# Yxxxb/LAVT-RS

Measured on AMD Instinct MI355X. Metric: train images/sec (480x480 Swin-B LAVT, fwd+bwd), higher is better.
Workload: dtype bf16; 1 GPU; swin_b_w12_480_b2; global_batch=2, image=480, n_l=20, parallelism=dp1, hip_graph=True, loss_kernel=fused upsample+CE

## Files before the change

lavt-rs_amd/csrc/gemm_tn_pipe.hip:

```cpp
#include "gemm_v2_helpers.h"
#include "internal.h"
#include "ln_bwd_body.h"

namespace {

typedef i32x8 __attribute__((aligned(4))) tnp_i32x8_u;
typedef __attribute__((address_space(4))) const tnp_i32x8_u* tnp_cptr8;
typedef __attribute__((address_space(4))) const int* tnp_cptr1;

template <int OFF> __device__ __forceinline__ void tnp_rd1(unsigned a, u64& d) {
    asm volatile("ds_read_b64_tr_b16 %0, %1 offset:%c2" : "=&v"(d) : "v"(a), "n"(OFF) : "memory");
}
__device__ __forceinline__ void tnp_tie1(u64& l, u64& h) { asm volatile("" : "+v"(l), "+v"(h)); }

constexpr int TNP_MAX = 6;
enum { TNP_ACCUMULATE = 1, TNP_COLSUM_ATOMIC = 2, TNP_NO_B = 4, TNP_VEC4 = 8, TNP_PART_VEC4 = 16, TNP_WT = 32 };
struct TnpMember {
    const bf16* A; const bf16* B; float* C; float* colsum;
    const int32_t* a_map; const int32_t* b_map; const float* a_rs;
    int64_t ldc;
    int lda, ldb, I, J, K, tiles_j, tile_end, rs_div, rs_n, flags;
    float alpha;
    float* part;
    int pieces, kt_per, tiles;
// ... 254 lines not shown
#undef TNP_MFMA_ONE

    const float alpha = m.alpha;
    const bool to_part = m.pieces > 1;
    float* const Cp = to_part ? m.part + (int64_t)piece * m.I * m.J : m.C;
    const int64_t ldc = to_part ? m.J : m.ldc;
    const bool accum = !to_part && (m.flags & TNP_ACCUMULATE), vec4 = to_part ? (m.flags & TNP_PART_VEC4) != 0 : (m.flags & TNP_VEC4) != 0;
    const bool wt = !to_part && (m.flags & TNP_WT) != 0;
    if (has_b) {
#pragma unroll
        for (int fi = 0; fi < 4; ++fi) {
            const int ii = i0 + wi * 64 + fi * 16 + l15;
#pragma unroll
            for (int fj = 0; fj < 2; ++fj) {
                const int jj = j0 + wj * 32 + fj * 16 + 4 * g4;
                if (ii < m.I && jj < m.J) {
                    float* dst = Cp + (int64_t)ii * ldc + jj;
                    float4 v = make_float4(alpha * acc[fi][fj][0], alpha * acc[fi][fj][1], alpha * acc[fi][fj][2], alpha * acc[fi][fj][3]);
                    if (vec4) {
                        if (accum) { const float4 o = *reinterpret_cast<const float4*>(dst); v.x += o.x; v.y += o.y; v.z += o.z; v.w += o.w; }
                        if (wt) st16_out(dst, make_uint4(__float_as_uint(v.x), __float_as_uint(v.y), __float_as_uint(v.z), __float_as_uint(v.w)));
                        else *reinterpret_cast<float4*>(dst) = v;
                    } else {
                        if (accum) { v.x += dst[0]; v.y += dst[1]; v.z += dst[2]; v.w += dst[3]; }
                        dst[0] = v.x; dst[1] = v.y; dst[2] = v.z; dst[3] = v.w;
                    }
                }
            }
        }
    }
    if (cs_wave && g4 == 0) {
        const bool cat = !to_part && ((m.flags & TNP_COLSUM_ATOMIC) || accum);
        float* const csb = to_part ? m.part + (int64_t)m.pieces * m.I * m.J + (int64_t)piece * m.I : m.colsum;
#pragma unroll
        for (int fi = 0; fi < 4; ++fi) {
            const int ii = i0 + wi * 64 + fi * 16 + l15;
            if (ii < m.I) {
                float* cs = csb + ii;
                if (cat) atomicAdd(cs, alpha * cacc[fi][0]); else *cs = alpha * cacc[fi][0];
            }
        }
    }
}

template <int STAGES, int LPR>
__global__ __launch_bounds__(512) void gemm_tn_pipe_kernel(const TnpGroup g, const TnpRider ln) {
    extern __shared__ __attribute__((aligned(16))) char smem[];
    const int bid = blockIdx.x;
    if (bid >= g.tiles) {
        if constexpr (LPR > 0) {
            int unit = 2 * (bid - g.tiles) + (int)(threadIdx.x >> 8);
            unit = unit < ln.blocks ? unit : ln.blocks - 1;
            layernorm_bwd_body<bf16, LPR, 1, 4, 0>(ln.dy, ln.x, nullptr, ln.gamma, ln.mean, ln.rstd, ln.dx, nullptr, nullptr, ln.partials, ln.dres, ln.rows, ln.C, nullptr,
                                                   nullptr, unit, ln.blocks, (int)(threadIdx.x & 255), reinterpret_cast<float*>(smem + (threadIdx.x >> 8) * 16384));
        }
        return;
    }
    const int t = bid;
    int k = 0;
    while (k + 1 < g.n && t >= g.m[k].tile_end) ++k;
    const TnpMember& m = g.m[k];
    const int local = t - (k ? g.m[k - 1].tile_end : 0);
    if ((m.a_map || m.b_map) && (m.K & 7)) tnp_tile<STAGES, 2>(m, local, smem);
    else if (m.a_map || m.b_map || m.a_rs) tnp_tile<STAGES, 1>(m, local, smem);
    else tnp_tile<STAGES, 0>(m, local, smem);
}

__global__ __launch_bounds__(256) void tnp_reduce_pieces(const TnpGroup g) {
    const TnpMember& m = g.m[blockIdx.y];
    const int ns = m.pieces;
    if (ns <= 1) return;
    const int64_t W = (int64_t)m.I * m.J, total = W + (m.colsum ? m.I : 0);
    const int64_t e0 = ((int64_t)blockIdx.x * 256 + threadIdx.x) * 4;
    if (e0 >= total) return;
    const bool no_b = (m.flags & TNP_NO_B) != 0;
    const bool v4 = !no_b && (m.flags & TNP_PART_VEC4) && (m.flags & TNP_VEC4) && (m.J % 4 == 0);
    if (v4 && e0 + 3 < W) {
        const float* q = m.part + e0;
        float4 a0 = make_float4(0.f, 0.f, 0.f, 0.f), a1 = a0, a2 = a0, a3 = a0;
        int s = 0;
        for (; s + 7 < ns; s += 8) {
            float4 v[8];
#pragma unroll
            for (int u = 0; u < 8; ++u) v[u] = *reinterpret_cast<const float4*>(q + (int64_t)(s + u) * W);
#pragma unroll
            for (int u = 0; u < 8; u += 4) {
                a0.x += v[u].x; a0.y += v[u].y; a0.z += v[u].z; a0.w += v[u].w; a1.x += v[u + 1].x; a1.y += v[u + 1].y; a1.z += v[u + 1].z; a1.w += v[u + 1].w;
                a2.x += v[u + 2].x; a2.y += v[u + 2].y; a2.z += v[u + 2].z; a2.w += v[u + 2].w; a3.x += v[u + 3].x; a3.y += v[u + 3].y; a3.z += v[u + 3].z; a3.w += v[u + 3].w;
            }
        }
        if (s < ns) {
            float4 v[7];
#pragma unroll
            for (int u = 0; u < 7; ++u) v[u] = *reinterpret_cast<const float4*>(q + (int64_t)min(s + u, ns - 1) * W);
#pragma unroll
            for (int u = 0; u < 7; ++u)
                if (s + u < ns) { a0.x += v[u].x; a0.y += v[u].y; a0.z += v[u].z; a0.w += v[u].w; }
        }
        const int64_t i = e0 / m.J;
        float4* c = reinterpret_cast<float4*>(m.C + i * m.ldc + (e0 - i * m.J));
        float4 o = *c;
        o.x += (a0.x + a1.x) + (a2.x + a3.x); o.y += (a0.y + a1.y) + (a2.y + a3.y); o.z += (a0.z + a1.z) + (a2.z + a3.z); o.w += (a0.w + a1.w) + (a2.w + a3.w);
        *c = o;
        return;
    }
    for (int k = 0; k < 4; ++k) {
        const int64_t e = e0 + k;
// ... 100 lines not shown
```

lavt-rs_amd/csrc/gemm_tn_v2.hip:

```cpp
#include "gemm_v2_helpers.h"
#include "internal.h"
#include "ln_bwd_body.h"

namespace {

__device__ __forceinline__ void dma4(const void* src, void* lds_dst) {
    __builtin_amdgcn_global_load_lds((gbl_void*)src, (lds_void*)lds_dst, 4, 0, 0);
}

struct TnOut {
    float* C;
    int64_t ldc;
    float* colsum;
    bool atomic, colsum_atomic;
};
template <int BI, int BJ, int WAVES, int STAGES, bool MAPS, int CS, bool CONVP = true>
__device__ __forceinline__ void tn_tile_range(const lavt_gemm_tn_t& p, const int tile_linear, const int bz, const int kt_begin, const int kt_end, const TnOut o, char* smem) {
    using T = bf16;
    constexpr int BK = 64, EPC = 8;
    constexpr int WAVES_I = 2, WAVES_J = WAVES / WAVES_I;
    constexpr int A_CH = BI / EPC, B_CH = BJ / EPC;
    constexpr int A_INSTR = BK * A_CH / (64 * WAVES), B_INSTR = BK * B_CH / (64 * WAVES);
    static_assert(A_INSTR * 64 * WAVES == BK * A_CH && B_INSTR * 64 * WAVES == BK * B_CH, "whole DMA instructions per operand tile");
    constexpr int A_BYTES = A_INSTR * WAVES * 1024, B_BYTES = B_INSTR * WAVES * 1024, STAGE_BYTES = A_BYTES + B_BYTES;
// ... 297 lines not shown
    const bool to_parts = p.partials != nullptr && nsplit > 1;
    float* const pbase = to_parts ? p.partials + (int64_t)bz * nsplit * ((int64_t)p.I * p.J + p.I) : nullptr;
    TnOut o;
    o.C = to_parts ? pbase + (int64_t)split_idx * p.I * p.J : p.C + (int64_t)bz * p.strideC;
    o.ldc = to_parts ? p.J : p.ldc;
    o.colsum = to_parts ? pbase + (int64_t)nsplit * p.I * p.J + (int64_t)split_idx * p.I : (p.colsum ? p.colsum + (int64_t)bz * p.strideColsum : nullptr);
    o.atomic = !to_parts && (nsplit > 1 || p.accumulate);
    o.colsum_atomic = p.colsum_atomic && !to_parts;
    tn_tile_range<BI, BJ, WAVES, STAGES, MAPS, CS, CONVP>(p, tile_linear, bz, kt_begin, kt_end, o, smem);
}

template <int BI, int BJ, int WAVES, int STAGES, bool MAPS, int CS, bool CONVP = true>
__global__ __launch_bounds__(WAVES * 64) void gemm_tn_v2_kernel(const lavt_gemm_tn_t p, int kt_per_split) {
    extern __shared__ __attribute__((aligned(16))) char smem[];
    tn_tile<BI, BJ, WAVES, STAGES, MAPS, CS, CONVP>(p, blockIdx.x, blockIdx.y, blockIdx.z, kt_per_split, gridDim.z, smem);
}

constexpr int TN_GROUP_MAX = 6;
struct TnGroup {
    lavt_gemm_tn_t p[TN_GROUP_MAX];
    int tile_end[TN_GROUP_MAX];
    int split[TN_GROUP_MAX];
    int n;
};
template <int BI, int BJ, int WAVES, int STAGES, bool MAPS, int CS>
__device__ __forceinline__ void grouped_tile(const TnGroup& g, const int bid, char* smem) {
    int k = 0;
    while (k + 1 < g.n && bid >= g.tile_end[k]) ++k;
    const int local = bid - (k ? g.tile_end[k - 1] : 0);
    const lavt_gemm_tn_t& p = g.p[k];
    const int ns = g.split[k], ktiles = (p.K + 63) / 64;
    if constexpr (MAPS) {
        if (!(p.a_rowmap || p.a_rowscale || p.b_rowmap)) {
            tn_tile<BI, BJ, WAVES, STAGES, false, CS, false>(p, local / ns, 0, local % ns, (ktiles + ns - 1) / ns, ns, smem);
            return;
        }
    }
    tn_tile<BI, BJ, WAVES, STAGES, MAPS, CS, false>(p, local / ns, 0, local % ns, (ktiles + ns - 1) / ns, ns, smem);
}
template <int BI, int BJ, int WAVES, int STAGES, bool MAPS, int CS>
__global__ __launch_bounds__(WAVES * 64, (BI == 128 && WAVES == 8) ? 4 : 1) void gemm_tn_v2_grouped_kernel(const TnGroup g) {
    extern __shared__ __attribute__((aligned(16))) char smem[];
    grouped_tile<BI, BJ, WAVES, STAGES, MAPS, CS>(g, blockIdx.x, smem);
}
struct LnRider {
    const bf16* dy; const bf16* x; const float* gamma; const float* mean; const float* rstd; bf16* dx; float* partials; const bf16* dres;
    int rows, C, blocks;
};
template <bool MAPS, int CS, int LPR, int CPL>
__global__ __launch_bounds__(256) void gemm_tn_v2_grouped_ln_kernel(const TnGroup g, const int tiles, const LnRider ln) {
    extern __shared__ __attribute__((aligned(16))) char smem[];
    if ((int)blockIdx.x >= tiles) {
        layernorm_bwd_body<bf16, LPR, CPL, 4, 0>(ln.dy, ln.x, nullptr, ln.gamma, ln.mean, ln.rstd, ln.dx, nullptr, nullptr, ln.partials, ln.dres, ln.rows, ln.C, nullptr,
                                                 nullptr, (int)blockIdx.x - tiles, ln.blocks, threadIdx.x, reinterpret_cast<float*>(smem));
        return;
    }
    grouped_tile<64, 64, 4, 2, MAPS, CS>(g, blockIdx.x, smem);
}

struct TnSk {
    int it_end[TN_GROUP_MAX];
    int kt[TN_GROUP_MAX];
    int tiles_end[TN_GROUP_MAX];
    int total, nw;
    float* slots;
};
template <int BI, int BJ, int WAVES, int STAGES, bool MAPS, int CS>
__global__ __launch_bounds__(WAVES * 64, (BI == 128 && WAVES == 8) ? 4 : 1) void gemm_tn_v2_streamk_kernel(const TnGroup g, const TnSk sk) {
    extern __shared__ __attribute__((aligned(16))) char smem[];
    const int w = blockIdx.x;
    const int lo = (int)((int64_t)w * sk.total / sk.nw), hi = (int)((int64_t)(w + 1) * sk.total / sk.nw);
    int seg = 0;
    for (int it = lo; it < hi; ++seg) {
        int m = 0;
        while (m + 1 < g.n && it >= sk.it_end[m]) ++m;
        const int ktm = sk.kt[m], local = it - (m ? sk.it_end[m - 1] : 0);
        const int tile = local / ktm, kb = local - tile * ktm, ke = min(ktm, kb + (hi - it));
        const lavt_gemm_tn_t& p = g.p[m];
        TnOut o;
        if (kb == 0 && ke == ktm) {
            o.C = p.C; o.ldc = p.ldc; o.colsum = p.colsum; o.atomic = p.accumulate != 0; o.colsum_atomic = p.colsum_atomic != 0;
        } else {
            const int tiles_j = (p.J + BJ - 1) / BJ, i0 = (tile / tiles_j) * BI, j0 = (tile % tiles_j) * BJ;
            float* slot = sk.slots + ((int64_t)w * 2 + (seg ? 1 : 0)) * (BI * BJ + BI);
            o.C = slot - (int64_t)i0 * BJ - j0; o.ldc = BJ; o.colsum = slot + BI * BJ - i0; o.atomic = false; o.colsum_atomic = false;
        }
        if (seg) __syncthreads();
        bool done = false;
        if constexpr (MAPS) {
            if (!(p.a_rowmap || p.a_rowscale || p.b_rowmap)) { tn_tile_range<BI, BJ, WAVES, STAGES, false, CS, false>(p, tile, 0, kb, ke, o, smem); done = true; }
        }
        if (!done) tn_tile_range<BI, BJ, WAVES, STAGES, MAPS, CS, false>(p, tile, 0, kb, ke, o, smem);
        it += ke - kb;
    }
}
template <int BI, int BJ>
__global__ __launch_bounds__(256) void tn_streamk_fixup(const TnGroup g, const TnSk sk) {
    int m = 0;
    while (m + 1 < g.n && (int)blockIdx.x >= sk.tiles_end[m]) ++m;
    const lavt_gemm_tn_t& p = g.p[m];
    const int tile = blockIdx.x - (m ? sk.tiles_end[m - 1] : 0), ktm = sk.kt[m];
    const int it0 = (m ? sk.it_end[m - 1] : 0) + tile * ktm, it1 = it0 + ktm;
    auto lo_of = [&](int w) { return (int)((int64_t)w * sk.total / sk.nw); };
    int w0 = (int)((int64_t)it0 * sk.nw / sk.total);
    while (w0 + 1 < sk.nw && lo_of(w0 + 1) <= it0) ++w0;
    while (w0 > 0 && lo_of(w0) > it0) --w0;
    int w1 = w0;
// ... 198 lines not shown
```

lavt-rs_amd/csrc/ln_bwd_body.h:

```cpp
#pragma once
#include "common.h"

namespace {

template <typename T>
__device__ __forceinline__ const T* ln_src(const T* x, const int32_t* gather, int64_t row, int C, int col, bool& ok) {
    if (!gather) { ok = true; return x + row * C + col; }
    const int cq = C >> 2, q = col / cq;
    const int src = gather[row * 4 + q];
    ok = src >= 0;
    return x + (int64_t)src * cq + (col - q * cq);
}

template <int LPR> __device__ __forceinline__ float group_sum(float v) {
#pragma unroll
    for (int o = LPR / 2; o > 0; o >>= 1) v += __shfl_xor(v, o, 64);
    return v;
}

template <typename T, int LPR, int CPL, int WAVES, int FLAGS = 3>
__device__ __forceinline__ void layernorm_bwd_body(const T* __restrict__ dy, const T* __restrict__ x,
                                                   const int32_t* __restrict__ gather, const float* __restrict__ gamma,
                                                   const float* __restrict__ mean, const float* __restrict__ rstd,
                                                   T* __restrict__ dx, float* __restrict__ dgamma, float* __restrict__ dbeta,
                                                   float* __restrict__ partials, const T* __restrict__ dres, int rows, int C,
                                                   T* __restrict__ xn_out_, const float* __restrict__ beta, const int bid, const int nblocks, const int tid, float* __restrict__ red) {
    if constexpr (!(FLAGS & 1)) gather = nullptr;
    T* const xn_out = (FLAGS & 2) ? xn_out_ : nullptr;
    constexpr int EPC = Chunk<T>::N, MAXC = CPL, RPW = 64 / LPR;
    const int lane = tid & 63, lir = lane % LPR, wave = tid >> 6;
    const int nchunk = C / EPC;
    constexpr int cpl = CPL;
    float dg[MAXC * EPC], db[MAXC * EPC];
#pragma unroll
    for (int e = 0; e < MAXC * EPC; ++e) { dg[e] = 0.f; db[e] = 0.f; }
    const int64_t rstride = (int64_t)nblocks * WAVES * RPW;
    for (int64_t row0 = ((int64_t)bid * WAVES + wave) * RPW; row0 < rows; row0 += rstride) {
        const int64_t row = row0 + lane / LPR;
        const bool live = row < rows;
        const float mu = live ? mean[row] : 0.f, rs = live ? rstd[row] : 0.f;
        float xh[MAXC * EPC], g[MAXC * EPC];
        constexpr bool RES_PRE = MAXC <= 2;
        uint4 rres[RES_PRE ? MAXC : 1];
        float s1 = 0.f, s2 = 0.f;
#pragma unroll
        for (int c = 0; c < MAXC; ++c) {
            const int ch = lir + LPR * c;
            const bool on = live && c < cpl && ch < nchunk;
            float fx[EPC], fg[EPC];
#pragma unroll
            for (int e = 0; e < EPC; ++e) { fx[e] = 0.f; fg[e] = 0.f; }
            if (on) {
                bool ok;
                const T* src = ln_src<T>(x, gather, row, C, ch * EPC, ok);
                if (ok) chunk_to_f<T>(*reinterpret_cast<const uint4*>(src), fx);
                chunk_to_f<T>(*reinterpret_cast<const uint4*>(dy + row * C + ch * EPC), fg);
                if constexpr (RES_PRE) { if (dres) rres[c] = *reinterpret_cast<const uint4*>(dres + row * C + ch * EPC); }
            }
#pragma unroll
            for (int e = 0; e < EPC; ++e) {
                const int k = c * EPC + e;
                xh[k] = on ? (fx[e] - mu) * rs : 0.f;
                const float gg = on ? fg[e] * gamma[ch * EPC + e] : 0.f;
                g[k] = gg;
                s1 += gg; s2 += gg * xh[k];
                dg[k] += fg[e] * xh[k];
                db[k] += fg[e];
            }
            if (xn_out && on) {
                float fy[EPC];
#pragma unroll
                for (int e = 0; e < EPC; ++e) fy[e] = xh[c * EPC + e] * gamma[ch * EPC + e] + beta[ch * EPC + e];
                *reinterpret_cast<uint4*>(xn_out + row * C + ch * EPC) = f_to_chunk<T>(fy);
            }
        }
        s1 = group_sum<LPR>(s1) / C; s2 = group_sum<LPR>(s2) / C;
#pragma unroll
        for (int c = 0; c < MAXC; ++c) {
            const int ch = lir + LPR * c;
            if (live && c < cpl && ch < nchunk) {
                float f[EPC];
#pragma unroll
                for (int e = 0; e < EPC; ++e) f[e] = rs * (g[c * EPC + e] - s1 - xh[c * EPC + e] * s2);
                if (dres) {
                    float fr[EPC];
                    if constexpr (RES_PRE) chunk_to_f<T>(rres[c], fr);
                    else chunk_to_f<T>(*reinterpret_cast<const uint4*>(dres + row * C + ch * EPC), fr);
#pragma unroll
                    for (int e = 0; e < EPC; ++e) f[e] += fr[e];
                }
                if (!gather) *reinterpret_cast<uint4*>(dx + row * C + ch * EPC) = f_to_chunk<T>(f);
                else {
                    const int cq = C >> 2, col = ch * EPC, qd = col / cq;
                    const int src = gather[row * 4 + qd];
                    if (src >= 0) *reinterpret_cast<uint4*>(dx + (int64_t)src * cq + (col - qd * cq)) = f_to_chunk<T>(f);
                }
            }
        }
    }
#pragma unroll
    for (int e = 0; e < MAXC * EPC; ++e) {
#pragma unroll
        for (int o = LPR; o < 64; o <<= 1) { dg[e] += __shfl_xor(dg[e], o, 64); db[e] += __shfl_xor(db[e], o, 64); }
    }
    constexpr int RW = LPR * CPL * EPC;
#pragma unroll
    for (int pass = 0; pass < 2; ++pass) {
        float* part = pass == 0 ? dg : db;
        float* dst = pass == 0 ? dgamma : dbeta;
        __syncthreads();
        if (wave > 0 && lane < LPR) {
#pragma unroll
            for (int c = 0; c < MAXC; ++c) {
                const int ch = lir + LPR * c;
                if (c < cpl && ch < nchunk)
#pragma unroll
                    for (int e = 0; e < EPC; ++e) red[(wave - 1) * RW + ch * EPC + e] = part[c * EPC + e];
            }
        }
        __syncthreads();
        if (wave == 0 && lane < LPR) {
#pragma unroll
            for (int c = 0; c < MAXC; ++c) {
                const int ch = lir + LPR * c;
                if (c < cpl && ch < nchunk)
#pragma unroll
                    for (int e = 0; e < EPC; ++e) {
                        const int col = ch * EPC + e;
                        float tot = part[c * EPC + e];
#pragma unroll
                        for (int w = 0; w < WAVES - 1; ++w) tot += red[w * RW + col];
                        if (partials) partials[((int64_t)bid * 2 + pass) * C + col] = tot;
                        else atomicAdd(dst + col, tot);
                    }
            }
        }
    }
}


}
```

lavt-rs_amd/csrc/norm.hip:

```cpp
#include <string.h>
#include "internal.h"
#include "fp8_pack.h"
#include "ln_bwd_body.h"
#include "dtable_body.h"

namespace {

constexpr int LN_MAXE = 32;

template <int EPC> __device__ __forceinline__ void ldc(const float* p, float* out) {
#pragma unroll
    for (int q = 0; q < EPC / 4; ++q) {
        const float4 v = *reinterpret_cast<const float4*>(p + 4 * q);
        out[4 * q] = v.x; out[4 * q + 1] = v.y; out[4 * q + 2] = v.z; out[4 * q + 3] = v.w;
    }
}

template <typename T, int LPR>
__global__ __launch_bounds__(256) void layernorm_fwd_kernel(const T* __restrict__ x, const int32_t* __restrict__ gather,
                                                            const float* __restrict__ gamma, const float* __restrict__ beta,
                                                            T* __restrict__ y, float* __restrict__ mean, float* __restrict__ rstd,
                                                            int rows, int C, float eps) {
    constexpr int EPC = Chunk<T>::N, MAXC = LPR == 64 ? LN_MAXE / EPC : 1, RPW = 64 / LPR;
    const int lane = threadIdx.x & 63, lir = lane % LPR;
    const int64_t row = ((int64_t)blockIdx.x * 4 + (threadIdx.x >> 6)) * RPW + lane / LPR;
    const bool live = row < rows;
    const int nchunk = C / EPC;
    float v[MAXC * EPC];
    float s = 0.f;
#pragma unroll
    for (int c = 0; c < MAXC; ++c) {
        const int ch = lir + LPR * c;
        float f[EPC];
#pragma unroll
        for (int e = 0; e < EPC; ++e) f[e] = 0.f;
        if (live && ch < nchunk) {
            bool ok;
            const T* src = ln_src<T>(x, gather, row, C, ch * EPC, ok);
            if (ok) chunk_to_f<T>(*reinterpret_cast<const uint4*>(src), f);
        }
#pragma unroll
        for (int e = 0; e < EPC; ++e) { v[c * EPC + e] = f[e]; s += f[e]; }
    }
    const float mu = group_sum<LPR>(s) / C;
    float q = 0.f;
#pragma unroll
    for (int c = 0; c < MAXC; ++c)
        if (lir + LPR * c < nchunk)
#pragma unroll
            for (int e = 0; e < EPC; ++e) { const float d = v[c * EPC + e] - mu; q += d * d; }
    const float rs = rsqrtf(group_sum<LPR>(q) / C + eps);
    if (!live) return;
    if (lir == 0) { mean[row] = mu; rstd[row] = rs; }
#pragma unroll
    for (int c = 0; c < MAXC; ++c) {
        const int ch = lir + LPR * c;
        if (ch < nchunk) {
            float f[EPC];
#pragma unroll
            for (int e = 0; e < EPC; ++e) f[e] = (v[c * EPC + e] - mu) * rs * gamma[ch * EPC + e] + beta[ch * EPC + e];
            *reinterpret_cast<uint4*>(y + row * C + ch * EPC) = f_to_chunk<T>(f);
        }
    }
}

template <typename T, int LPR, int CPL, int WAVES, int FLAGS = 3>
__global__ __launch_bounds__(WAVES * 64) void layernorm_bwd_kernel(const T* __restrict__ dy, const T* __restrict__ x,
                                                            const int32_t* __restrict__ gather, const float* __restrict__ gamma,
                                                            const float* __restrict__ mean, const float* __restrict__ rstd,
                                                            T* __restrict__ dx, float* __restrict__ dgamma, float* __restrict__ dbeta,
                                                            float* __restrict__ partials, const T* __restrict__ dres, int rows, int C,
                                                            T* __restrict__ xn_out_, const float* __restrict__ beta) {
    __shared__ float red[(WAVES - 1) * (LPR * CPL * Chunk<T>::N)];
    layernorm_bwd_body<T, LPR, CPL, WAVES, FLAGS>(dy, x, gather, gamma, mean, rstd, dx, dgamma, dbeta, partials, dres, rows, C, xn_out_, beta, blockIdx.x, gridDim.x,
                                                  threadIdx.x, red);
}

struct DtableRider {
    const bf16* slab; float* part;
    int slab_ld, wd, wh, ww, nwin, N, heads, rows_per_block, win_per_group, gx, gz;
};
template <typename T, int LPR, int CPL, int FLAGS>
__global__ __launch_bounds__(256) void layernorm_bwd_dtable_kernel(const T* __restrict__ dy, const T* __restrict__ x, const float* __restrict__ gamma,
                                                                   const float* __restrict__ mean, const float* __restrict__ rstd, T* __restrict__ dx,
                                                                   float* __restrict__ partials, const T* __restrict__ dres, int rows, int C,
                                                                   T* __restrict__ xn_out_, const float* __restrict__ beta, const int ln_blocks, const DtableRider job) {
    extern __shared__ __attribute__((aligned(16))) char dsm[];
    __shared__ float red[3 * (LPR * CPL * Chunk<T>::N)];
    if ((int)blockIdx.x >= ln_blocks) {
        const int u = (int)blockIdx.x - ln_blocks;
        const int bx = u % job.gx, hh = (u / job.gx) % job.heads, bz = u / (job.gx * job.heads);
        dtable_block(job.slab, job.part, job.slab_ld, job.wd, job.wh, job.ww, job.nwin, job.N, job.heads, job.rows_per_block, job.win_per_group, bx, hh, bz, job.gx,
                     threadIdx.x, dsm);
        return;
    }
    layernorm_bwd_body<T, LPR, CPL, 4, FLAGS>(dy, x, nullptr, gamma, mean, rstd, dx, nullptr, nullptr, partials, dres, rows, C, xn_out_, beta, blockIdx.x, ln_blocks,
                                              threadIdx.x, red);
}

__global__ __launch_bounds__(256) void reduce_partials_kernel(const float* __restrict__ partials, int nblk, int W, int C,
                                                              float* __restrict__ o1, float* __restrict__ o2) {
    __shared__ float red[8][33];
    const int col = threadIdx.x & 31, slice = threadIdx.x >> 5;
    const int w = blockIdx.x * 32 + col;
    const int per = (nblk + gridDim.y - 1) / gridDim.y, k0 = blockIdx.y * per, k1 = min(nblk, k0 + per);
    float a = 0.f, a1 = 0.f, a2 = 0.f, a3 = 0.f;
    if (w < W) {
        int k = k0 + slice;
        for (; k + 24 < k1; k += 32) {
            a += partials[(int64_t)k * W + w]; a1 += partials[(int64_t)(k + 8) * W + w];
            a2 += partials[(int64_t)(k + 16) * W + w]; a3 += partials[(int64_t)(k + 24) * W + w];
        }
        for (; k < k1; k += 8) a += partials[(int64_t)k * W + w];
    }
    red[slice][col] = (a + a1) + (a2 + a3);
    __syncthreads();
    if (slice == 0 && w < W && k0 < k1) {
        float t = 0.f;
#pragma unroll
        for (int k = 0; k < 8; ++k) t += red[k][col];
        const int g2 = w / C, c = w - g2 * C;
        float* dst = (g2 & 1) ? o2 : o1;
        if (gridDim.y > 1) atomicAdd(dst + (int64_t)(g2 >> 1) * C + c, t);
        else dst[(int64_t)(g2 >> 1) * C + c] += t;
    }
}
constexpr int RPM_COLS = 128;
template <bool COMPACT>
__global__ __launch_bounds__(256) void reduce_partials_multi_kernel(const int64_t* __restrict__ desc, int nsets) {
    int set = blockIdx.z, cb = blockIdx.x;
    if constexpr (COMPACT) {
        const int ln = threadIdx.x & 63;
        int nb = ln < nsets ? (2 * (int)desc[(int64_t)ln * 5 + 2] + RPM_COLS - 1) / RPM_COLS : 0;
        int pre = nb;
#pragma unroll
        for (int o = 1; o < 64; o <<= 1) {
            const int up = __shfl_up(pre, o, 64);
            if (ln >= o) pre += up;
        }
        const unsigned long long hit = __ballot(pre > (int)blockIdx.x);
        set = hit ? __ffsll((long long)hit) - 1 : nsets - 1;
        const int before = __shfl(pre - nb, set, 64);
        cb = (int)blockIdx.x - before;
    }
    const int64_t* d = desc + (int64_t)set * 5;
    const float* partials = reinterpret_cast<const float*>(d[0]);
    const int nblk = (int)d[1], C = (int)d[2], W = 2 * C;
    float* o1 = reinterpret_cast<float*>(d[3]);
    float* o2 = reinterpret_cast<float*>(d[4]);
    if (cb * RPM_COLS >= W) return;
// ... 419 lines not shown
                for (int e = 0; e < EPC; ++e) q_m = fmaxf(q_m, fabsf(fg[e]));
            }
            if (mul && dmul) *reinterpret_cast<uint4*>(dmul + off) = f_to_chunk<T>(fdm);
        }
    }
    if constexpr (AMAX) q8_block_amax(q_m, amax);
}

static int apply_rows_per_block(int rows, int groups, int C, int epc) {
    const int cpr = C / epc, span = cpr < 256 ? cpr : 256, rstep = 256 / span;
    int rpb = cdiv((long)rows * groups, 1024);
    if (rpb < 8 * rstep) rpb = 8 * rstep;
    return rpb;
}

inline int ew_grid(int64_t n) { int64_t b = (n + 255) / 256; return (int)(b < 1 ? 1 : (b > 4096 ? 4096 : b)); }

}

#define DISPATCH_T(dtype, NAME, ...)                                   \
    if (dtype == LAVT_F32) { using T = float; __VA_ARGS__; }           \
    else if (dtype == LAVT_BF16) { using T = bf16; __VA_ARGS__; }      \
    else { lavt_set_error(NAME ": bad dtype %d", dtype); return LAVT_ERR_INVALID; }

extern "C" int lavt_layernorm_fwd(int dtype, const void* x, const int32_t* gather, const float* gamma, const float* beta, void* y,
                                  float* mean, float* rstd, int rows, int C, float eps, void* stream) {
    const int epc = dtype == LAVT_F32 ? 4 : 8;
    LAVT_CHECK_ARG(x && gamma && beta && y && mean && rstd && rows > 0, "lavt_layernorm_fwd: bad arguments");
    LAVT_CHECK_ARG(C > 0 && C <= 2048 && C % epc == 0 && (!gather || (C / 4) % epc == 0), "lavt_layernorm_fwd: unsupported C=%d", C);
    hipStream_t st = reinterpret_cast<hipStream_t>(stream);
    const int nchunk = C / epc;
#define LN_FWD(LPR_) hipLaunchKernelGGL((layernorm_fwd_kernel<T, LPR_>), dim3(cdiv(rows, 4 * (64 / LPR_))), dim3(256), 0, st, (const T*)x, gather, gamma, beta, (T*)y, mean, rstd, rows, C, eps)
    DISPATCH_T(dtype, "lavt_layernorm_fwd", if (nchunk <= 16) LN_FWD(16); else if (nchunk <= 32) LN_FWD(32); else LN_FWD(64));
#undef LN_FWD
    LAVT_CHECK_LAUNCH("lavt_layernorm_fwd");
    return LAVT_OK;
}

static int ln_bwd_geometry(int dtype, int rows, int C, int* lpr_out, int* cpl_out, int* waves_out) {
    const int epc = dtype == LAVT_F32 ? 4 : 8;
    const int nchunk = C / epc;
    const int lpr = nchunk <= 16 ? 16 : nchunk <= 32 ? 32 : 64;
    const int cpl = cdiv(nchunk, lpr);
    const int waves = 4;
    const int rpb = 4 * (64 / lpr);
    int blocks = cdiv(rows, rpb);
    if (blocks > 1280) blocks = cdiv(rows, 2 * rpb);
    if (blocks > 2048) blocks = 2048;
    if (blocks < 1) blocks = 1;
    *lpr_out = lpr; *cpl_out = cpl;
    if (waves_out) *waves_out = waves;
    return blocks;
}
extern "C" int lavt_layernorm_bwd_blocks(int dtype, int rows, int C) { int a, b; return ln_bwd_geometry(dtype, rows, C, &a, &b, nullptr); }
int lavt_ln_bwd_geometry(int dtype, int rows, int C, int* lpr, int* cpl, int* waves) { return ln_bwd_geometry(dtype, rows, C, lpr, cpl, waves); }

static int layernorm_bwd_impl(int dtype, const void* dy, const void* x, const int32_t* gather, const float* gamma,
                              const float* mean, const float* rstd, void* dx, float* dgamma, float* dbeta, float* ws, int64_t ws_floats,
                              const void* dres, int rows, int C, void* stream, bool partial_only, void* xn_out = nullptr, const float* beta = nullptr) {
    const int epc = dtype == LAVT_F32 ? 4 : 8;
    LAVT_CHECK_ARG(dy && x && gamma && mean && rstd && dx && (partial_only || (dgamma && dbeta)) && rows > 0, "lavt_layernorm_bwd: bad arguments");
    LAVT_CHECK_ARG(C > 0 && C <= 2048 && C % epc == 0 && (!gather || (C / 4) % epc == 0), "lavt_layernorm_bwd: unsupported C=%d", C);
    LAVT_CHECK_ARG(!(gather && dres), "lavt_layernorm_bwd: dres is not supported together with gather");
    hipStream_t st = reinterpret_cast<hipStream_t>(stream);
    int lpr, cpl, waves;
    const int blocks = ln_bwd_geometry(dtype, rows, C, &lpr, &cpl, &waves);
    float* partials = (ws && ws_floats >= (int64_t)blocks * 2 * C) ? ws : nullptr;
    LAVT_CHECK_ARG(!partial_only || partials, "lavt_layernorm_bwd_partial: scratch of %ld floats needed", (long)blocks * 2 * C);
#define LN_BWD_F(LPR_, CPL_, WV_, F_) hipLaunchKernelGGL((layernorm_bwd_kernel<T, LPR_, CPL_, WV_, F_>), dim3(blocks), dim3(WV_ * 64), 0, st, (const T*)dy, (const T*)x, gather, gamma, mean, rstd, (T*)dx, dgamma, dbeta, partials, (const T*)dres, rows, C, (T*)xn_out, beta)
#define LN_BWD(LPR_, CPL_, WV_) do { if (gather) LN_BWD_F(LPR_, CPL_, WV_, 1); else if (xn_out) LN_BWD_F(LPR_, CPL_, WV_, 2); else LN_BWD_F(LPR_, CPL_, WV_, 0); } while (0)
    DISPATCH_T(dtype, "lavt_layernorm_bwd",
               if (lpr == 16) LN_BWD(16, 1, 4); else if (lpr == 32) LN_BWD(32, 1, 4);
               else if (cpl == 1) LN_BWD(64, 1, 4); else if (cpl == 2) LN_BWD(64, 2, 4); else if (cpl <= 4) LN_BWD(64, 4, 4); else LN_BWD(64, 8, 4));
#undef LN_BWD
#undef LN_BWD_F
    if (partials && !partial_only) hipLaunchKernelGGL(reduce_partials_kernel, reduce_partials_grid(blocks, 2 * C), dim3(256), 0, st, partials, blocks, 2 * C, C, dgamma, dbeta);
    LAVT_CHECK_LAUNCH("lavt_layernorm_bwd");
    return LAVT_OK;
}
extern "C" int lavt_layernorm_bwd(int dtype, const void* dy, const void* x, const int32_t* gather, const float* gamma,
                                  const float* mean, const float* rstd, void* dx, float* dgamma, float* dbeta, float* ws, int64_t ws_floats,
                                  const void* dres, int rows, int C, void* stream) {
    return layernorm_bwd_impl(dtype, dy, x, gather, gamma, mean, rstd, dx, dgamma, dbeta, ws, ws_floats, dres, rows, C, stream, false);
}
extern "C" int lavt_layernorm_bwd_partial(int dtype, const void* dy, const void* x, const int32_t* gather, const float* gamma, const float* mean,
                                          const float* rstd, void* dx, float* ws, int64_t ws_floats, const void* dres, int rows, int C, void* stream) {
    return layernorm_bwd_impl(dtype, dy, x, gather, gamma, mean, rstd, dx, nullptr, nullptr, ws, ws_floats, dres, rows, C, stream, true);
}
int lavt_layernorm_bwd_partial_impl(int dtype, const void* dy, const void* x, const float* gamma, const float* mean, const float* rstd, void* dx, float* ws,
                                    int64_t ws_floats, const void* dres, int rows, int C, void* stream) {
    return layernorm_bwd_impl(dtype, dy, x, nullptr, gamma, mean, rstd, dx, nullptr, nullptr, ws, ws_floats, dres, rows, C, stream, true);
}
extern "C" int lavt_layernorm_bwd_partial_xn(int dtype, const void* dy, const void* x, const float* gamma, const float* beta, const float* mean, const float* rstd,
                                             void* dx, void* xn, float* ws, int64_t ws_floats, const void* dres, int rows, int C, void* stream) {
    LAVT_CHECK_ARG(xn && beta, "lavt_layernorm_bwd_partial_xn: xn and beta required");
    return layernorm_bwd_impl(dtype, dy, x, nullptr, gamma, mean, rstd, dx, nullptr, nullptr, ws, ws_floats, dres, rows, C, stream, true, xn, beta);
}
extern "C" int lavt_layernorm_bwd_partial_xn_dtable(int dtype, const void* dy, const void* x, const float* gamma, const float* beta, const float* mean, const float* rstd,
                                                    void* dx, void* xn, float* ws, int64_t ws_floats, const void* dres, int rows, int C, const lavt_dtable_job_t* job, void* stream) {
    LAVT_CHECK_ARG(dy && x && gamma && mean && rstd && dx && ws && job && rows > 0 && ((xn != nullptr) == (beta != nullptr)), "lavt_layernorm_bwd_partial_xn_dtable: bad arguments");
    int lpr, cpl, waves;
    const int blocks = ln_bwd_geometry(dtype, rows, C, &lpr, &cpl, &waves);
    if (dtype != LAVT_BF16 || waves != 4 || cpl > 2 || C % 8 || ws_floats < (int64_t)blocks * 2 * C) return 1;
    static_assert(sizeof(DtableRider) == sizeof(lavt_dtable_job_t), "lavt_dtable_job_t mirrors DtableRider");
    DtableRider r;
    memcpy(&r, job, sizeof(r));
    const int R = (2 * r.wd - 1) * (2 * r.wh - 1) * (2 * r.ww - 1);
    const size_t lds = (size_t)(R + r.N) * 4 + 16;
    const int riders = r.gx * r.heads * r.gz;
    hipStream_t st = reinterpret_cast<hipStream_t>(stream);
    using T = bf16;
#define LN_BWD_DT_F(LPR_, CPL_, F_) hipLaunchKernelGGL((layernorm_bwd_dtable_kernel<T, LPR_, CPL_, F_>), dim3(blocks + riders), dim3(256), lds, st, (const T*)dy, (const T*)x, gamma, mean, rstd, (T*)dx, ws, (const T*)dres, rows, C, (T*)xn, beta, blocks, r)
#define LN_BWD_DT(LPR_, CPL_) do { if (xn) LN_BWD_DT_F(LPR_, CPL_, 2); else LN_BWD_DT_F(LPR_, CPL_, 0); } while (0)
    if (lpr == 16) LN_BWD_DT(16, 1); else if (lpr == 32) LN_BWD_DT(32, 1); else if (cpl == 1) LN_BWD_DT(64, 1); else LN_BWD_DT(64, 2);
#undef LN_BWD_DT
#undef LN_BWD_DT_F
    LAVT_CHECK_LAUNCH("lavt_layernorm_bwd_partial_xn_dtable");
    return LAVT_OK;
}
extern "C" int lavt_layernorm_bwd_xn(int dtype, const void* dy, const void* x, const float* gamma, const float* beta, const float* mean, const float* rstd,
                                     void* dx, void* xn, float* dgamma, float* dbeta, float* ws, int64_t ws_floats, const void* dres, int rows, int C, void* stream) {
    LAVT_CHECK_ARG(xn && beta, "lavt_layernorm_bwd_xn: xn and beta required");
    return layernorm_bwd_impl(dtype, dy, x, nullptr, gamma, mean, rstd, dx, dgamma, dbeta, ws, ws_floats, dres, rows, C, stream, false, xn, beta);
}
extern "C" int lavt_reduce_partials_column_blocks(int C) { return (2 * C + RPM_COLS - 1) / RPM_COLS; }
extern "C" int lavt_reduce_partials_multi(const int64_t* desc, int n, int total_column_blocks, void* stream) {
    LAVT_CHECK_ARG(desc && n > 0, "lavt_reduce_partials_multi: bad arguments");
    if (total_column_blocks > 0 && n <= 64)
        hipLaunchKernelGGL(reduce_partials_multi_kernel<true>, dim3(total_column_blocks, 8, 1), dim3(256), 0, reinterpret_cast<hipStream_t>(stream), desc, n);
    else
        hipLaunchKernelGGL(reduce_partials_multi_kernel<false>, dim3(4096 / RPM_COLS, 8, n), dim3(256), 0, reinterpret_cast<hipStream_t>(stream), desc, n);
    LAVT_CHECK_LAUNCH("lavt_reduce_partials_multi");
    return LAVT_OK;
}
extern "C" int64_t lavt_reduce_partials_det_stage(int W) { return (int64_t)RP_DET_MAX_SLICES * W; }
extern "C" int lavt_reduce_partials_det(const float* partials, int nblk, int W, int C, float* o1, float* o2, float* stage, int64_t stage_floats, void* stream) {
    LAVT_CHECK_ARG(partials && o1 && o2 && nblk > 0 && C > 0 && W > 0 && W % (2 * C) == 0, "lavt_reduce_partials_det: bad arguments");
    reduce_partials_det(partials, nblk, W, C, o1, o2, stage_floats >= (int64_t)RP_DET_MAX_SLICES * W ? stage : nullptr, reinterpret_cast<hipStream_t>(stream));
    LAVT_CHECK_LAUNCH("lavt_reduce_partials_det");
    return LAVT_OK;
}
extern "C" int lavt_reduce_partials_multi_det(const int64_t* desc, int n, int total_column_blocks, float* stage, int64_t stage_floats, void* stream) {
    constexpr int slices = 8;
    LAVT_CHECK_ARG(desc && n > 0 && n <= 64 && total_column_blocks > 0 && stage && stage_floats >= (int64_t)total_column_blocks * slices * RPM_COLS,
                   "lavt_reduce_partials_multi_det: n <= 64 sets, their column-block total and a stage of total_column_blocks * 8 * 128 floats required");
    hipStream_t st = reinterpret_cast<hipStream_t>(stream);
    hipLaunchKernelGGL(reduce_partials_multi_det_kernel<false>, dim3(total_column_blocks, slices), dim3(256), 0, st, desc, n, stage, slices);
    hipLaunchKernelGGL(reduce_partials_multi_det_kernel<true>, dim3(total_column_blocks), dim3(RPM_COLS), 0, st, desc, n, stage, slices);
    LAVT_CHECK_LAUNCH("lavt_reduce_partials_multi_det");
    return LAVT_OK;
}

static int stats_launch_geometry(int rows, int groups, int C, int epc, int* rows_per_block) {
    const int cpr = C / epc, span = cpr < 256 ? cpr : 256, rstep = 256 / span;
    if (groups < 1) groups = 1;
    int t = 8;
    while (t > 2 && (long)cdiv(rows, t * rstep) * groups < 256) t >>= 1;
    int rpb = t * rstep;
    const int cap = 1024 / groups > 0 ? 1024 / groups : 1;
    if (cdiv(rows, rpb) > cap) rpb = cdiv(cdiv(rows, cap), rstep) * rstep;
    *rows_per_block = rpb;
    return cdiv(rows, rpb);
}

extern "C" int lavt_colstats(int dtype, const void* x, float* sum, float* sumsq, float* ws, int64_t ws_floats, int groups, int rows, int C, void* stream) {
// ... 165 lines not shown
```

Before: 269.9 images/s.

## Persist LayerNorm backward blocks with prefetch and LDS tree column reduction

Caps the LayerNorm backward grid at 512 workgroups and makes them loop over rows grid-stride. For CPL<=2 the next row's x, dy, residual and statistics are prefetched into registers, and gamma and beta are hoisted out of the row loop. The dgamma/dbeta reduction replaces the cross-lane shuffles plus serial wave-0 sum with a per-slot LDS dump that all threads sum in parallel. Because fewer blocks now write partials, the unused partial rows are zeroed so the downstream reducer's row count stays the same. The cost is more register pressure, more LDS, and extra zero writes.

```diff
diff --git a/lavt-rs_amd/csrc/gemm_tn_pipe.hip b/lavt-rs_amd/csrc/gemm_tn_pipe.hip
--- a/lavt-rs_amd/csrc/gemm_tn_pipe.hip
+++ b/lavt-rs_amd/csrc/gemm_tn_pipe.hip
@@ -330,7 +330,7 @@
             int unit = 2 * (bid - g.tiles) + (int)(threadIdx.x >> 8);
             unit = unit < ln.blocks ? unit : ln.blocks - 1;
             layernorm_bwd_body<bf16, LPR, 1, 4, 0>(ln.dy, ln.x, nullptr, ln.gamma, ln.mean, ln.rstd, ln.dx, nullptr, nullptr, ln.partials, ln.dres, ln.rows, ln.C, nullptr,
-                                                   nullptr, unit, ln.blocks, (int)(threadIdx.x & 255), reinterpret_cast<float*>(smem + (threadIdx.x >> 8) * 16384));
+                                                   nullptr, unit, ln.blocks, ln.blocks, (int)(threadIdx.x & 255), reinterpret_cast<float*>(smem + (threadIdx.x >> 8) * 16384));
         }
         return;
     }
diff --git a/lavt-rs_amd/csrc/gemm_tn_v2.hip b/lavt-rs_amd/csrc/gemm_tn_v2.hip
--- a/lavt-rs_amd/csrc/gemm_tn_v2.hip
+++ b/lavt-rs_amd/csrc/gemm_tn_v2.hip
@@ -373,7 +373,7 @@
     extern __shared__ __attribute__((aligned(16))) char smem[];
     if ((int)blockIdx.x >= tiles) {
         layernorm_bwd_body<bf16, LPR, CPL, 4, 0>(ln.dy, ln.x, nullptr, ln.gamma, ln.mean, ln.rstd, ln.dx, nullptr, nullptr, ln.partials, ln.dres, ln.rows, ln.C, nullptr,
-                                                 nullptr, (int)blockIdx.x - tiles, ln.blocks, threadIdx.x, reinterpret_cast<float*>(smem));
+                                                 nullptr, (int)blockIdx.x - tiles, ln.blocks, ln.blocks, threadIdx.x, reinterpret_cast<float*>(smem));
         return;
     }
     grouped_tile<64, 64, 4, 2, MAPS, CS>(g, blockIdx.x, smem);
diff --git a/lavt-rs_amd/csrc/ln_bwd_body.h b/lavt-rs_amd/csrc/ln_bwd_body.h
--- a/lavt-rs_amd/csrc/ln_bwd_body.h
+++ b/lavt-rs_amd/csrc/ln_bwd_body.h
@@ -18,13 +18,45 @@
     return v;
 }
 
+template <int CPL> struct LnTrip {
+    static constexpr bool RES_PRE = CPL <= 2;
+    uint4 x[CPL], dy[CPL], res[RES_PRE ? CPL : 1];
+    float mu, rs;
+};
+
+template <typename T, int LPR, int CPL>
+__device__ __forceinline__ void ln_trip_load(LnTrip<CPL>& t, const T* __restrict__ dy, const T* __restrict__ x, const int32_t* __restrict__ gather,
+                                             const float* __restrict__ mean, const float* __restrict__ rstd, const T* __restrict__ dres, const int64_t row0, const int rows,
+                                             const int C, const int lane) {
+    constexpr int EPC = Chunk<T>::N;
+    const int lir = lane % LPR, nchunk = C / EPC;
+    const int64_t row = row0 + lane / LPR;
+    const bool live = row < rows;
+    t.mu = live ? mean[row] : 0.f; t.rs = live ? rstd[row] : 0.f;
+#pragma unroll
+    for (int c = 0; c < CPL; ++c) {
+        const int ch = lir + LPR * c;
+        t.x[c] = make_uint4(0u, 0u, 0u, 0u); t.dy[c] = make_uint4(0u, 0u, 0u, 0u);
+        if (live && ch < nchunk) {
+            bool ok;
+            const T* src = ln_src<T>(x, gather, row, C, ch * EPC, ok);
+            if (ok) t.x[c] = *reinterpret_cast<const uint4*>(src);
+            t.dy[c] = *reinterpret_cast<const uint4*>(dy + row * C + ch * EPC);
+            if constexpr (LnTrip<CPL>::RES_PRE) { if (dres) t.res[c] = *reinterpret_cast<const uint4*>(dres + row * C + ch * EPC); }
+        }
+    }
+}
+
+template <typename T, int CPL, int WAVES> constexpr int LN_BWD_RED_FLOATS = WAVES * 64 * 2 * Chunk<T>::N * (CPL < 2 ? CPL : 2);
+
 template <typename T, int LPR, int CPL, int WAVES, int FLAGS = 3>
 __device__ __forceinline__ void layernorm_bwd_body(const T* __restrict__ dy, const T* __restrict__ x,
                                                    const int32_t* __restrict__ gather, const float* __restrict__ gamma,
                                                    const float* __restrict__ mean, const float* __restrict__ rstd,
                                                    T* __restrict__ dx, float* __restrict__ dgamma, float* __restrict__ dbeta,
                                                    float* __restrict__ partials, const T* __restrict__ dres, int rows, int C,
-                                                   T* __restrict__ xn_out_, const float* __restrict__ beta, const int bid, const int nblocks, const int tid, float* __restrict__ red) {
+                                                   T* __restrict__ xn_out_, const float* __restrict__ beta, const int bid, const int nblocks, const int prows, const int tid,
+                                                   float* __restrict__ red) {
     if constexpr (!(FLAGS & 1)) gather = nullptr;
     T* const xn_out = (FLAGS & 2) ? xn_out_ : nullptr;
     constexpr int EPC = Chunk<T>::N, MAXC = CPL, RPW = 64 / LPR;
@@ -35,33 +67,46 @@
 #pragma unroll
     for (int e = 0; e < MAXC * EPC; ++e) { dg[e] = 0.f; db[e] = 0.f; }
     const int64_t rstride = (int64_t)nblocks * WAVES * RPW;
-    for (int64_t row0 = ((int64_t)bid * WAVES + wave) * RPW; row0 < rows; row0 += rstride) {
+    constexpr bool RES_PRE = LnTrip<CPL>::RES_PRE, TWO = CPL <= 2;
+    constexpr bool GB_PRE = CPL <= 2;
+    float gam[GB_PRE ? MAXC * EPC : 1], bet[GB_PRE ? MAXC * EPC : 1];
+    if constexpr (GB_PRE) {
+#pragma unroll
+        for (int c = 0; c < MAXC; ++c) {
+            const int ch = lir + LPR * c;
+#pragma unroll
+            for (int e = 0; e < EPC; ++e) {
+                gam[c * EPC + e] = ch < nchunk ? gamma[ch * EPC + e] : 0.f;
+                bet[c * EPC + e] = (xn_out && ch < nchunk) ? beta[ch * EPC + e] : 0.f;
+            }
+        }
+    }
+    const int64_t first = ((int64_t)bid * WAVES + wave) * RPW;
+    LnTrip<CPL> nxt;
+    if constexpr (TWO) { if (first < rows) ln_trip_load<T, LPR, CPL>(nxt, dy, x, gather, mean, rstd, dres, first, rows, C, lane); }
+    for (int64_t row0 = first; row0 < rows; row0 += rstride) {
+        LnTrip<CPL> cur;
+        if constexpr (TWO) {
+            cur = nxt;
+            if (row0 + rstride < rows) ln_trip_load<T, LPR, CPL>(nxt, dy, x, gather, mean, rstd, dres, row0 + rstride, rows, C, lane);
+        } else ln_trip_load<T, LPR, CPL>(cur, dy, x, gather, mean, rstd, dres, row0, rows, C, lane);
         const int64_t row = row0 + lane / LPR;
         const bool live = row < rows;
-        const float mu = live ? mean[row] : 0.f, rs = live ? rstd[row] : 0.f;
+        const float mu = cur.mu, rs = cur.rs;
         float xh[MAXC * EPC], g[MAXC * EPC];
-        constexpr bool RES_PRE = MAXC <= 2;
-        uint4 rres[RES_PRE ? MAXC : 1];
         float s1 = 0.f, s2 = 0.f;
 #pragma unroll
         for (int c = 0; c < MAXC; ++c) {
             const int ch = lir + LPR * c;
             const bool on = live && c < cpl && ch < nchunk;
             float fx[EPC], fg[EPC];
-#pragma unroll
-            for (int e = 0; e < EPC; ++e) { fx[e] = 0.f; fg[e] = 0.f; }
-            if (on) {
-                bool ok;
-                const T* src = ln_src<T>(x, gather, row, C, ch * EPC, ok);
-                if (ok) chunk_to_f<T>(*reinterpret_cast<const uint4*>(src), fx);
-                chunk_to_f<T>(*reinterpret_cast<const uint4*>(dy + row * C + ch * EPC), fg);
-                if constexpr (RES_PRE) { if (dres) rres[c] = *reinterpret_cast<const uint4*>(dres + row * C + ch * EPC); }
-            }
+            chunk_to_f<T>(cur.x[c], fx);
+            chunk_to_f<T>(cur.dy[c], fg);
 #pragma unroll
             for (int e = 0; e < EPC; ++e) {
                 const int k = c * EPC + e;
                 xh[k] = on ? (fx[e] - mu) * rs : 0.f;
-                const float gg = on ? fg[e] * gamma[ch * EPC + e] : 0.f;
+                const float gg = on ? fg[e] * (GB_PRE ? gam[k] : gamma[ch * EPC + e]) : 0.f;
                 g[k] = gg;
                 s1 += gg; s2 += gg * xh[k];
                 dg[k] += fg[e] * xh[k];
@@ -70,7 +115,7 @@
             if (xn_out && on) {
                 float fy[EPC];
 #pragma unroll
-                for (int e = 0; e < EPC; ++e) fy[e] = xh[c * EPC + e] * gamma[ch * EPC + e] + beta[ch * EPC + e];
+                for (int e = 0; e < EPC; ++e) fy[e] = xh[c * EPC + e] * (GB_PRE ? gam[c * EPC + e] : gamma[ch * EPC + e]) + (GB_PRE ? bet[c * EPC + e] : beta[ch * EPC + e]);
                 *reinterpret_cast<uint4*>(xn_out + row * C + ch * EPC) = f_to_chunk<T>(fy);
             }
         }
@@ -84,7 +129,7 @@
                 for (int e = 0; e < EPC; ++e) f[e] = rs * (g[c * EPC + e] - s1 - xh[c * EPC + e] * s2);
                 if (dres) {
                     float fr[EPC];
-                    if constexpr (RES_PRE) chunk_to_f<T>(rres[c], fr);
+                    if constexpr (RES_PRE) chunk_to_f<T>(cur.res[c], fr);
                     else chunk_to_f<T>(*reinterpret_cast<const uint4*>(dres + row * C + ch * EPC), fr);
 #pragma unroll
                     for (int e = 0; e < EPC; ++e) f[e] += fr[e];
@@ -98,41 +143,35 @@
             }
         }
     }
+    constexpr int CPP = CPL < 2 ? CPL : 2, PW = CPP * LPR * EPC, NSLOT = WAVES * RPW;
+    static_assert(NSLOT * 2 * PW == LN_BWD_RED_FLOATS<T, CPL, WAVES>, "the lent LDS");
+    const int slot = wave * RPW + lane / LPR;
 #pragma unroll
-    for (int e = 0; e < MAXC * EPC; ++e) {
+    for (int c0 = 0; c0 < CPL; c0 += CPP) {
+        __syncthreads();
 #pragma unroll
-        for (int o = LPR; o < 64; o <<= 1) { dg[e] += __shfl_xor(dg[e], o, 64); db[e] += __shfl_xor(db[e], o, 64); }
-    }
-    constexpr int RW = LPR * CPL * EPC;
+        for (int cc = 0; cc < CPP; ++cc) {
+            float* pg = red + (slot * 2 + 0) * PW + cc * LPR * EPC + lir * EPC;
+            float* pb = red + (slot * 2 + 1) * PW + cc * LPR * EPC + lir * EPC;
 #pragma unroll
-    for (int pass = 0; pass < 2; ++pass) {
-        float* part = pass == 0 ? dg : db;
-        float* dst = pass == 0 ? dgamma : dbeta;
-        __syncthreads();
-        if (wave > 0 && lane < LPR) {
-#pragma unroll
-            for (int c = 0; c < MAXC; ++c) {
-                const int ch = lir + LPR * c;
-                if (c < cpl && ch < nchunk)
-#pragma unroll
-                    for (int e = 0; e < EPC; ++e) red[(wave - 1) * RW + ch * EPC + e] = part[c * EPC + e];
+            for (int e = 0; e < EPC; e += 4) {
+                const int k = (c0 + cc) * EPC + e;
+                *reinterpret_cast<float4*>(pg + e) = make_float4(dg[k], dg[k + 1], dg[k + 2], dg[k + 3]);
+                *reinterpret_cast<float4*>(pb + e) = make_float4(db[k], db[k + 1], db[k + 2], db[k + 3]);
             }
         }
         __syncthreads();
-        if (wave == 0 && lane < LPR) {
 #pragma unroll
-            for (int c = 0; c < MAXC; ++c) {
-                const int ch = lir + LPR * c;
-                if (c < cpl && ch < nchunk)
+        for (int o = tid; o < 2 * PW; o += WAVES * 64) {
+            const int which = o / PW, j = o - which * PW, col = c0 * LPR * EPC + j;
+            if (col < C) {
+                float tot = red[which * PW + j];
 #pragma unroll
-                    for (int e = 0; e < EPC; ++e) {
-                        const int col = ch * EPC + e;
-                        float tot = part[c * EPC + e];
-#pragma unroll
-                        for (int w = 0; w < WAVES - 1; ++w) tot += red[w * RW + col];
-                        if (partials) partials[((int64_t)bid * 2 + pass) * C + col] = tot;
-                        else atomicAdd(dst + col, tot);
-                    }
+                for (int s = 1; s < NSLOT; ++s) tot += red[(s * 2 + which) * PW + j];
+                if (partials) {
+                    partials[((int64_t)bid * 2 + which) * C + col] = tot;
+                    for (int64_t pr = (int64_t)bid + nblocks; pr < prows; pr += nblocks) partials[(pr * 2 + which) * C + col] = 0.f;
+                } else atomicAdd((which ? dbeta : dgamma) + col, tot);
             }
         }
     }
diff --git a/lavt-rs_amd/csrc/norm.hip b/lavt-rs_amd/csrc/norm.hip
--- a/lavt-rs_amd/csrc/norm.hip
+++ b/lavt-rs_amd/csrc/norm.hip
@@ -70,10 +70,10 @@
                                                             const float* __restrict__ mean, const float* __restrict__ rstd,
                                                             T* __restrict__ dx, float* __restrict__ dgamma, float* __restrict__ dbeta,
                                                             float* __restrict__ partials, const T* __restrict__ dres, int rows, int C,
-                                                            T* __restrict__ xn_out_, const float* __restrict__ beta) {
-    __shared__ float red[(WAVES - 1) * (LPR * CPL * Chunk<T>::N)];
+                                                            T* __restrict__ xn_out_, const float* __restrict__ beta, const int prows) {
+    __shared__ __attribute__((aligned(16))) float red[LN_BWD_RED_FLOATS<T, CPL, WAVES>];
     layernorm_bwd_body<T, LPR, CPL, WAVES, FLAGS>(dy, x, gather, gamma, mean, rstd, dx, dgamma, dbeta, partials, dres, rows, C, xn_out_, beta, blockIdx.x, gridDim.x,
-                                                  threadIdx.x, red);
+                                                  prows, threadIdx.x, red);
 }
 
 struct DtableRider {
@@ -84,9 +84,10 @@
 __global__ __launch_bounds__(256) void layernorm_bwd_dtable_kernel(const T* __restrict__ dy, const T* __restrict__ x, const float* __restrict__ gamma,
                                                                    const float* __restrict__ mean, const float* __restrict__ rstd, T* __restrict__ dx,
                                                                    float* __restrict__ partials, const T* __restrict__ dres, int rows, int C,
-                                                                   T* __restrict__ xn_out_, const float* __restrict__ beta, const int ln_blocks, const DtableRider job) {
+                                                                   T* __restrict__ xn_out_, const float* __restrict__ beta, const int ln_blocks, const int prows,
+                                                                   const DtableRider job) {
     extern __shared__ __attribute__((aligned(16))) char dsm[];
-    __shared__ float red[3 * (LPR * CPL * Chunk<T>::N)];
+    __shared__ __attribute__((aligned(16))) float red[LN_BWD_RED_FLOATS<T, CPL, 4>];
     if ((int)blockIdx.x >= ln_blocks) {
         const int u = (int)blockIdx.x - ln_blocks;
         const int bx = u % job.gx, hh = (u / job.gx) % job.heads, bz = u / (job.gx * job.heads);
@@ -95,7 +96,7 @@
         return;
     }
     layernorm_bwd_body<T, LPR, CPL, 4, FLAGS>(dy, x, nullptr, gamma, mean, rstd, dx, nullptr, nullptr, partials, dres, rows, C, xn_out_, beta, blockIdx.x, ln_blocks,
-                                              threadIdx.x, red);
+                                              prows, threadIdx.x, red);
 }
 
 __global__ __launch_bounds__(256) void reduce_partials_kernel(const float* __restrict__ partials, int nblk, int W, int C,
@@ -621,6 +622,10 @@
     if (waves_out) *waves_out = waves;
     return blocks;
 }
+static int ln_bwd_launch_blocks(int prows) {
+    constexpr int cap = 512;
+    return prows < cap ? prows : cap;
+}
 extern "C" int lavt_layernorm_bwd_blocks(int dtype, int rows, int C) { int a, b; return ln_bwd_geometry(dtype, rows, C, &a, &b, nullptr); }
 int lavt_ln_bwd_geometry(int dtype, int rows, int C, int* lpr, int* cpl, int* waves) { return ln_bwd_geometry(dtype, rows, C, lpr, cpl, waves); }
 
@@ -634,9 +639,10 @@
     hipStream_t st = reinterpret_cast<hipStream_t>(stream);
     int lpr, cpl, waves;
     const int blocks = ln_bwd_geometry(dtype, rows, C, &lpr, &cpl, &waves);
+    const int wgs = ln_bwd_launch_blocks(blocks);
     float* partials = (ws && ws_floats >= (int64_t)blocks * 2 * C) ? ws : nullptr;
     LAVT_CHECK_ARG(!partial_only || partials, "lavt_layernorm_bwd_partial: scratch of %ld floats needed", (long)blocks * 2 * C);
-#define LN_BWD_F(LPR_, CPL_, WV_, F_) hipLaunchKernelGGL((layernorm_bwd_kernel<T, LPR_, CPL_, WV_, F_>), dim3(blocks), dim3(WV_ * 64), 0, st, (const T*)dy, (const T*)x, gather, gamma, mean, rstd, (T*)dx, dgamma, dbeta, partials, (const T*)dres, rows, C, (T*)xn_out, beta)
+#define LN_BWD_F(LPR_, CPL_, WV_, F_) hipLaunchKernelGGL((layernorm_bwd_kernel<T, LPR_, CPL_, WV_, F_>), dim3(wgs), dim3(WV_ * 64), 0, st, (const T*)dy, (const T*)x, gather, gamma, mean, rstd, (T*)dx, dgamma, dbeta, partials, (const T*)dres, rows, C, (T*)xn_out, beta, blocks)
 #define LN_BWD(LPR_, CPL_, WV_) do { if (gather) LN_BWD_F(LPR_, CPL_, WV_, 1); else if (xn_out) LN_BWD_F(LPR_, CPL_, WV_, 2); else LN_BWD_F(LPR_, CPL_, WV_, 0); } while (0)
     DISPATCH_T(dtype, "lavt_layernorm_bwd",
                if (lpr == 16) LN_BWD(16, 1, 4); else if (lpr == 32) LN_BWD(32, 1, 4);
@@ -671,6 +677,7 @@
     int lpr, cpl, waves;
     const int blocks = ln_bwd_geometry(dtype, rows, C, &lpr, &cpl, &waves);
     if (dtype != LAVT_BF16 || waves != 4 || cpl > 2 || C % 8 || ws_floats < (int64_t)blocks * 2 * C) return 1;
+    const int wgs = ln_bwd_launch_blocks(blocks);
     static_assert(sizeof(DtableRider) == sizeof(lavt_dtable_job_t), "lavt_dtable_job_t mirrors DtableRider");
     DtableRider r;
     memcpy(&r, job, sizeof(r));
@@ -679,7 +686,7 @@
     const int riders = r.gx * r.heads * r.gz;
     hipStream_t st = reinterpret_cast<hipStream_t>(stream);
     using T = bf16;
-#define LN_BWD_DT_F(LPR_, CPL_, F_) hipLaunchKernelGGL((layernorm_bwd_dtable_kernel<T, LPR_, CPL_, F_>), dim3(blocks + riders), dim3(256), lds, st, (const T*)dy, (const T*)x, gamma, mean, rstd, (T*)dx, ws, (const T*)dres, rows, C, (T*)xn, beta, blocks, r)
+#define LN_BWD_DT_F(LPR_, CPL_, F_) hipLaunchKernelGGL((layernorm_bwd_dtable_kernel<T, LPR_, CPL_, F_>), dim3(wgs + riders), dim3(256), lds, st, (const T*)dy, (const T*)x, gamma, mean, rstd, (T*)dx, ws, (const T*)dres, rows, C, (T*)xn, beta, wgs, blocks, r)
 #define LN_BWD_DT(LPR_, CPL_) do { if (xn) LN_BWD_DT_F(LPR_, CPL_, 2); else LN_BWD_DT_F(LPR_, CPL_, 0); } while (0)
     if (lpr == 16) LN_BWD_DT(16, 1); else if (lpr == 32) LN_BWD_DT(32, 1); else if (cpl == 1) LN_BWD_DT(64, 1); else LN_BWD_DT(64, 2);
 #undef LN_BWD_DT
```

Result: no change. 270.9 images/s, median of 6 (+0.4%).
